# xingyizhou/CenterTrack

Hardware: NVIDIA H100
Metric: frames/sec (device-timed) DLA-34 512x512 (higher is better)
Workload: dtype bf16

## Files before the change

### centertrack_b200/csrc/conv_halo.cu

```cuda
#include "conv_common.cuh"
#include "wgmma.cuh"
#include <cuda.h>
#include <stdlib.h>
#include <string.h>

namespace ctb {

constexpr int HT_W = 8, HT_H = 16;

__device__ unsigned long long* g_halo_trace = nullptr;
__device__ __forceinline__ unsigned long long* h_trace_ptr() {
  unsigned long long* t = g_halo_trace;
  return (t != nullptr && blockIdx.x == 0) ? t : nullptr;
}
__device__ __forceinline__ void h_stamp(unsigned long long* t, int it, int k) {
  if (t != nullptr && it < 256) t[it * 8 + k] = (unsigned long long)clock64();
}
constexpr int H_THREADS = 288;
constexpr int H_MMA_WARPS = 8;
constexpr int H_STAGING_BYTES = 2 * 64 * EPI_PITCH * 4;

struct HaloArgs {
  ConvGeom g;
  const __nv_bfloat16* w;
  const float* shift;
  const __nv_bfloat16* residual;
  void* out;
  int n_tile, n_tiles_n, nblk, planes, pw, ph, plane_bytes, box_bytes, halo_stages;
  int tw, th;
  int tiles_x, tiles_y, tiles_total;
  int pair_taps;
  int swz;
  int merged_xc;
  int out_s2d;
  int sum3;
  uint32_t w_bytes;
  int m_nky, m_nkx, m_nc, m_nq;
  uint32_t m_sky, m_skx, m_sc, m_sq, m_alo, m_ahi;
};

template <int N, bool OVERLAP>
__global__ void __launch_bounds__(H_THREADS, (N <= 128 && !OVERLAP) ? 2 : 1)
conv_halo_kernel(const HaloArgs a, const __grid_constant__ CUtensorMap tmap) {
  extern __shared__ __align__(1024) unsigned char hsm_dyn[];
  unsigned char* sm = hsm_dyn + ((1024u - (smem_u32(hsm_dyn) & 1023u)) & 1023u);
  const ConvGeom& g = a.g;
  const int tid = threadIdx.x, warp = tid >> 5, lane = tid & 31;
  unsigned long long* const trace = h_trace_ptr();
  const int S = a.halo_stages;
  const uint32_t halo_bytes = (uint32_t)a.planes * a.plane_bytes;

  const uint32_t base = smem_u32(sm);
  const uint32_t sW = base;
  const uint32_t sH = base + ((a.w_bytes + 1023u) & ~1023u);
  const uint32_t off_stg = ((a.w_bytes + 1023u) & ~1023u) + S * halo_bytes;
  const uint32_t off_bar = off_stg + H_STAGING_BYTES;
  const uint32_t bars = base + off_bar;
  const uint32_t w_full = bars;
  auto halo_full = [&](int s) { return bars + 8u * (1 + s); };
  auto halo_empty = [&](int s) { return bars + 8u * (1 + S + s); };

  pdl_trigger();
  if (tid == 0) {
    mbar_init(w_full, 1);
    for (int s = 0; s < S; ++s) { mbar_init(halo_full(s), 1); mbar_init(halo_empty(s), H_MMA_WARPS); }
    mbar_init_fence();
  }
  float* s_shift = reinterpret_cast<float*>(sm + off_bar + 256);
  {
    const int n0s = (blockIdx.x % a.n_tiles_n) * N;
    for (int j = tid; j < 256; j += H_THREADS)
      s_shift[j] = (a.shift && j < N && n0s + j < g.C_out) ? __ldg(a.shift + n0s + j) : 0.f;
  }
  __syncthreads();
  if (warp == 8 && lane == 0) {
    mbar_arrive_expect_tx(w_full, a.w_bytes);
    bulk_g2s(sW, reinterpret_cast<const unsigned char*>(a.w) + (size_t)(blockIdx.x % a.n_tiles_n) * a.w_bytes, a.w_bytes, w_full);
  }
  pdl_wait();

  const int nt = blockIdx.x % a.n_tiles_n;
  const int sp0 = blockIdx.x / a.n_tiles_n;
  const int sp_stride = gridDim.x / a.n_tiles_n;
  const int sp_total = a.tiles_total;
  const int n0 = nt * N;
  const int per_img = a.tiles_x * a.tiles_y;

  if (warp == 8) {
    if (lane == 0) {
      int it = 0;
      for (int sp = sp0; sp < sp_total; sp += sp_stride, ++it) {
        const int s = it % S;
        const uint32_t ph = (uint32_t)(it / S) & 1u;
        mbar_wait(halo_empty(s), ph ^ 1u, 1, it);
        h_stamp(trace, it, 0);
        const int b = sp / per_img, r = sp - b * per_img;
        const int ty = r / a.tiles_x, tx = r - ty * a.tiles_x;
        const int x0 = tx * a.tw - g.pad, y0 = ty * a.th - g.pad;
        mbar_arrive_expect_tx(halo_full(s), (uint32_t)(a.planes * a.box_bytes));
        if (a.merged_xc) {
          tma_3d(sH + s * halo_bytes, &tmap, x0 * 8, y0, b, halo_full(s));
        } else {
          const int cstep = a.swz ? (a.swz >> 1) : 8;
          for (int p = 0; p < a.planes; ++p)
            tma_4d(sH + s * halo_bytes + p * a.plane_bytes, &tmap, p * cstep, x0, y0, b, halo_full(s));
        }
        h_stamp(trace, it, 1);
      }
    }
  } else {
    const int wg = warp >> 2, w4 = warp & 3;
    const int lrow = 32 * (w4 & 1) + lane;
    const int chalf = w4 >> 1;
    const int row = 64 * wg + lrow;
    const uint32_t stg = base + off_stg + (uint32_t)wg * (64u * EPI_PITCH * 4u);
    const uint64_t b_desc0 = wg_desc(sW, (uint32_t)N * 16u, 128u, 0u);
    const uint32_t b_step = ((uint32_t)N * 32u) >> 4;
    const uint32_t half16 = (uint32_t)wg * 8u * (a.m_ahi & 0x3FFFu);
    const int gpr = a.tw >> 3;
    const int gy = (row >> 3) / gpr, rx = (((row >> 3) % gpr) << 3) | (row & 7);
    const int HWo = g.OH * g.OW;
    constexpr int PF = 2;
    uint4 rq[PF][2];
    const bool use_res = a.residual != nullptr && g.out_mode == CT_OUT_NHWC && !a.sum3;
    auto prefetch_residual = [&](int sp_n) {
      const int bn = sp_n / per_img, rn = sp_n - bn * per_img;
      const int tyn = rn / a.tiles_x, txn = rn - tyn * a.tiles_x;
      const int oyn = tyn * a.th + gy, oxn = txn * a.tw + rx;
      const bool okn = oyn < g.OH && oxn < g.OW;
      const size_t pn = ((size_t)bn * g.OH + oyn) * g.OW + oxn;
#pragma unroll
      for (int i = 0; i < PF; ++i) {
        const int col = chalf * 16 + 32 * i;
        rq[i][0] = make_uint4(0, 0, 0, 0); rq[i][1] = make_uint4(0, 0, 0, 0);
        if (okn && col < N && n0 + col < g.C_out) {
          const uint4* rp = reinterpret_cast<const uint4*>(a.residual + pn * g.ld_res + n0 + col);
          rq[i][0] = __ldg(rp); rq[i][1] = __ldg(rp + 1);
        }
      }
    };
    if (use_res && sp0 < sp_total) prefetch_residual(sp0);
    mbar_wait(w_full, 0, 2, 0);
    if constexpr (OVERLAP)
      if (wg == 1 && sp0 < sp_total) named_arrive(3, 256);
    float acc[N / 2];
    int it = 0;
    for (int sp = sp0; sp < sp_total; sp += sp_stride, ++it) {
      const int s = it % S;
      const uint32_t ph = (uint32_t)(it / S) & 1u;
      if constexpr (OVERLAP) named_sync(3 + wg, 256);
      mbar_wait(halo_full(s), ph, 3, it);
      if (tid == 0) h_stamp(trace, it, 2);
      const uint32_t a_lo0 = a.m_alo + (sH >> 4) + ((uint32_t)s * halo_bytes >> 4) + half16;
      uint64_t b_desc = b_desc0;
      uint32_t accum = 0;
      wg_fence();
      for (int ky = 0; ky < a.m_nky; ++ky)
        for (int kx = 0; kx < a.m_nkx; ++kx)
          for (int c = 0; c < a.m_nc; ++c)
            for (int qq = 0; qq < a.m_nq; ++qq) {
              const uint32_t a_lo = a_lo0 + (uint32_t)ky * a.m_sky + (uint32_t)kx * a.m_skx + (uint32_t)c * a.m_sc +
                                    (uint32_t)qq * a.m_sq;
              Wgmma<N>::mma(acc, ((uint64_t)a.m_ahi << 32) | (uint64_t)a_lo, b_desc, accum);
              accum = 1;
              b_desc += b_step;
            }
      wg_commit();
      wg_wait<0>();
      wg_fence_operand(acc);
      if constexpr (OVERLAP) named_arrive(3 + (wg ^ 1), 256);
      __syncwarp();
      if (lane == 0) mbar_arrive(halo_empty(s));
      if (tid == 0) h_stamp(trace, it, 4);

      const int b = sp / per_img, r = sp - b * per_img;
      const int ty = r / a.tiles_x, tx = r - ty * a.tiles_x;
      const int oy = ty * a.th + gy, ox = tx * a.tw + rx;
      const bool p_ok = oy < g.OH && ox < g.OW;
      const size_t p = a.out_s2d ? ((((size_t)b * (g.OH >> 1) + (oy >> 1)) * (g.OW >> 1) + (ox >> 1)) << 2) + (((oy & 1) << 1) | (ox & 1))
                                 : ((size_t)b * g.OH + oy) * g.OW + ox;
      if (tid == 0) h_stamp(trace, it, 5);
      float s8[8];
#pragma unroll
      for (int j = 0; j < 8; ++j) s8[j] = 0.f;
#pragma unroll
      for (int c0 = 0; c0 < N; c0 += 32) {
        named_sync(1 + wg, 128);
        stage_acc_chunk(acc, c0, stg, 0);
        named_sync(1 + wg, 128);
        const uint32_t srow = stg + (uint32_t)lrow * EPI_PITCH * 4u;
        if (a.sum3) {
#pragma unroll
          for (int grp = 0; grp < 3; ++grp) {
            if (grp * 16 < c0 || grp * 16 >= c0 + 32 || grp * 16 >= N) continue;
            if (!((a.sum3 >> grp) & 1)) continue;
            float rr[8];
            lds_f(srow + (uint32_t)(grp * 16 - c0 + chalf * 8) * 4u, rr);
            const float4* sh4 = reinterpret_cast<const float4*>(s_shift + grp * 16 + chalf * 8);
            const float4 sa = sh4[0], sb = sh4[1];
            s8[0] += fmaxf(rr[0] + sa.x, 0.f); s8[1] += fmaxf(rr[1] + sa.y, 0.f);
            s8[2] += fmaxf(rr[2] + sa.z, 0.f); s8[3] += fmaxf(rr[3] + sa.w, 0.f);
            s8[4] += fmaxf(rr[4] + sb.x, 0.f); s8[5] += fmaxf(rr[5] + sb.y, 0.f);
            s8[6] += fmaxf(rr[6] + sb.z, 0.f); s8[7] += fmaxf(rr[7] + sb.w, 0.f);
          }
          continue;
        }
        const int col = c0 + chalf * 16;
        const int o0 = n0 + col;
        if (col >= N || !p_ok || o0 >= g.C_out) continue;
        float v[16];
        lds_f(srow + (uint32_t)chalf * 64u, v);
        const float4* sh4 = reinterpret_cast<const float4*>(s_shift + col);
#pragma unroll
        for (int j4 = 0; j4 < 4; ++j4) {
          const float4 sh = sh4[j4];
          v[4 * j4 + 0] += sh.x; v[4 * j4 + 1] += sh.y; v[4 * j4 + 2] += sh.z; v[4 * j4 + 3] += sh.w;
        }
        if (g.out_mode == CT_OUT_NHWC) {
          if (a.residual) {
            uint4 ra, rb;
            const int ci = col >> 5;
            if (ci < PF) {
// ... 56 lines not shown
    if ((g.OH | g.OW) & 1 || d->residual)
      return fail(CT_ERR_INVALID, "conv_halo: CT_OUT_NHWC_S2D needs even OH / OW, no residual%s", "");
    a.out_s2d = 1;
    a.g.out_mode = CT_OUT_NHWC;
  }
  if (a.sum3 && !(g.C_out == 48 && n_tile == 48 && g.out_mode == CT_OUT_NHWC && d->shift))
    return fail(CT_ERR_INVALID, "conv_halo: sum3 epilogue needs C_out == n_tile == 48, NHWC output, shift%s", "");
  if (g.out_mode == CT_OUT_NHWC && !a.sum3 && (g.C_out % 16 != 0 || g.ld_out % 8 != 0))
    return fail(CT_ERR_INVALID, "conv_halo: NHWC bf16 output needs C_out %% 16 == 0, ld_out %% 8 == 0%s", "");
  if (d->residual && (g.out_mode != CT_OUT_NHWC || g.ld_res % 8 != 0))
    return fail(CT_ERR_INVALID, "conv_halo: residual only for NHWC bf16 outputs, ld_res %% 8 == 0%s", "");
  a.n_tile = n_tile;
  a.n_tiles_n = (g.C_out + n_tile - 1) / n_tile;
  a.pair_taps = g.C_in == 8;
  a.nblk = halo_blocks(g.C_in, g.KH, g.KW);
  if (a.nblk > 160) return fail(CT_ERR_UNSUPPORTED, "conv_halo: more than 160 K=16 blocks per tile%s (%ld)", "", (long)a.nblk);
  static const bool force_planes = [] { const char* e = getenv("CTB_HALO_MODE"); return e && strcmp(e, "planes") == 0; }();
  a.swz = (g.C_in > 64) ? 128 : ((!force_planes && (g.C_in == 16 || g.C_in == 32 || g.C_in == 64)) ? g.C_in * 2 : 0);
  a.merged_xc = (g.C_in == 8 && g.ld_in == 8) ? 1 : 0;
  a.planes = a.swz ? (g.C_in * 2 + a.swz - 1) / a.swz : g.C_in / 8;
  a.tw = HT_W; a.th = HT_H;
  static const int wide_env = getenv("CTB_HALO_WIDE") ? atoi(getenv("CTB_HALO_WIDE")) : 1;
  if (wide_env && g.KH == 1 && g.KW == 1 && g.out_mode == CT_OUT_NCHW_F32 && a.swz && g.OW % 32 == 0 && g.OH % 4 == 0) {
    a.tw = 32; a.th = 4;
  }
  a.pw = a.tw + g.KW - 1 + (a.pair_taps ? 1 : 0);
  a.ph = a.th + g.KH - 1;
  a.box_bytes = a.pw * a.ph * (a.swz ? a.swz : 16);
  a.plane_bytes = (a.box_bytes + 1023) / 1024 * 1024;
  a.w_bytes = (uint32_t)a.nblk * n_tile * 32u;
  if (a.pair_taps) {
    a.m_nky = g.KH; a.m_nkx = (g.KW + 1) / 2; a.m_nc = 1; a.m_nq = 1;
    a.m_sky = a.pw; a.m_skx = 2; a.m_sc = 0; a.m_sq = 0;
    a.m_alo = 1u << 16;
    a.m_ahi = (uint32_t)a.pw;
  } else if (a.swz) {
    const uint32_t rb16 = (uint32_t)a.swz >> 4;
    a.m_nky = g.KH; a.m_nkx = g.KW; a.m_nc = a.planes; a.m_nq = (g.C_in < 64 ? g.C_in : 64) / 16;
    a.m_sky = (uint32_t)a.pw * rb16; a.m_skx = rb16; a.m_sc = (uint32_t)a.plane_bytes >> 4; a.m_sq = 2;
    a.m_alo = 1u << 16;
    const uint32_t layout = a.swz == 128 ? 1u : (a.swz == 64 ? 2u : 3u);
    const uint32_t sbo16 = a.tw == HT_W ? (uint32_t)a.pw * rb16 : 8u * rb16;
    a.m_ahi = sbo16 | (layout << 30);
  } else {
    a.m_nky = g.KH; a.m_nkx = g.KW; a.m_nc = 1; a.m_nq = g.C_in / 16;
    a.m_sky = a.pw; a.m_skx = 1; a.m_sc = 0; a.m_sq = 2u * ((uint32_t)a.plane_bytes >> 4);
    a.m_alo = ((uint32_t)a.plane_bytes >> 4) << 16;
    a.m_ahi = (uint32_t)a.pw;
  }
  a.tiles_x = (g.OW + a.tw - 1) / a.tw;
  a.tiles_y = (g.OH + a.th - 1) / a.th;
  a.tiles_total = g.B * a.tiles_x * a.tiles_y;
  const size_t halo_bytes = (size_t)a.planes * a.plane_bytes;
  auto smem_for = [&](int s) { return (size_t)((a.w_bytes + 1023) & ~1023u) + s * halo_bytes + H_STAGING_BYTES + 256 + 1024 + 1024; };
  auto ctas_for = [&](int s) {
    const int n = (int)((227 * 1024) / smem_for(s));
    return n > 2 ? 2 : n;
  };
  int stages = 2;
  for (int sdeep = 4; sdeep >= 3; --sdeep)
    if (smem_for(sdeep) <= 227 * 1024 && ctas_for(sdeep) == ctas_for(2)) { stages = sdeep; break; }
  static const int stages_env = getenv("CTB_HALO_STAGES") ? atoi(getenv("CTB_HALO_STAGES")) : 0;
  if (stages_env >= 2) stages = stages_env;
  if (smem_for(stages) > 227 * 1024)
    return fail(CT_ERR_UNSUPPORTED, "conv_halo: weights + halo do not fit in shared memory%s (%ld bytes)", "",
                (long)smem_for(stages));
  a.halo_stages = stages;
  int per_sm = ctas_for(stages);
  if (n_tile > 128) per_sm = 1;
  static const int overlap_env = getenv("CTB_HALO_OVERLAP") ? atoi(getenv("CTB_HALO_OVERLAP")) : 1;
  c.smem_bytes = (int32_t)smem_for(stages);
  c.stages = stages;
  c.tile_w = a.tw;
  c.tile_h = a.th;
  c.ctas_per_sm = per_sm;
  c.overlap = overlap_env && per_sm == 1 && n_tile >= 64 && n_tile <= 128;
  return CT_OK;
}

int conv_config_halo(const ct_conv_desc* d, ConvConfig* c) {
  HaloArgs a;
  return halo_config(d, a, *c);
}

int conv_forward_halo(const ct_conv_desc* d, cudaStream_t st) {
  HaloArgs a;
  ConvConfig c;
  const int rc = halo_config(d, a, c);
  if (rc != CT_OK) return rc;
  if (((uintptr_t)d->x & 15) || ((uintptr_t)d->w & 15) || ((uintptr_t)d->out & 15) || ((uintptr_t)d->residual & 15))
    return fail(CT_ERR_INVALID, "conv_halo: x/w/out/residual must be 16-byte aligned%s", "");
  a.w = (const __nv_bfloat16*)d->w;
  a.shift = d->shift;
  a.residual = (const __nv_bfloat16*)d->residual;
  a.out = d->out;
  const ConvGeom& g = a.g;

  CUtensorMap tmap;
  int r;
  if (a.merged_xc) {
    const cuuint64_t dims[3] = {(cuuint64_t)g.W * 8, (cuuint64_t)g.H, (cuuint64_t)g.B};
    const cuuint64_t strides[2] = {(cuuint64_t)g.W * 16, (cuuint64_t)g.H * g.W * 16};
    const cuuint32_t box[3] = {(cuuint32_t)a.pw * 8, (cuuint32_t)a.ph, 1};
    r = encode_tmap_bf16(&tmap, d->x, 3, dims, strides, box, CU_TENSOR_MAP_SWIZZLE_NONE);
  } else {
    const cuuint64_t dims[4] = {(cuuint64_t)g.C_in, (cuuint64_t)g.W, (cuuint64_t)g.H, (cuuint64_t)g.B};
    const cuuint64_t strides[3] = {(cuuint64_t)g.ld_in * 2, (cuuint64_t)g.W * g.ld_in * 2,
                                   (cuuint64_t)g.H * g.W * g.ld_in * 2};
    const cuuint32_t box[4] = {(cuuint32_t)(a.swz ? a.swz / 2 : 8), (cuuint32_t)a.pw, (cuuint32_t)a.ph, 1};
    const CUtensorMapSwizzle sw = a.swz == 128 ? CU_TENSOR_MAP_SWIZZLE_128B
                                  : a.swz == 64 ? CU_TENSOR_MAP_SWIZZLE_64B
                                  : a.swz == 32 ? CU_TENSOR_MAP_SWIZZLE_32B : CU_TENSOR_MAP_SWIZZLE_NONE;
    r = encode_tmap_bf16(&tmap, d->x, 4, dims, strides, box, sw);
  }
  if (r != CT_OK) return r;

  const int sms = device_sm_count();
  long want = (long)sms * c.ctas_per_sm;
  long groups = want / a.n_tiles_n;
  if (groups < 1) groups = 1;
  if (groups > a.tiles_total) groups = a.tiles_total;
  const int grid = (int)(groups * a.n_tiles_n);
  return dispatch_n_tile(a.n_tile, [&](auto n) {
    constexpr int NT = decltype(n)::value;
    if constexpr (NT >= 64 && NT <= 128)
      if (c.overlap)
        return launch_big_smem<conv_halo_kernel<NT, true>>(dim3(grid), dim3(H_THREADS), c.smem_bytes, st, a, tmap);
    return launch_big_smem<conv_halo_kernel<NT, false>>(dim3(grid), dim3(H_THREADS), c.smem_bytes, st, a, tmap);
  });
}

}
```

### centertrack_b200/csrc/conv_heads.cu

```cuda
#include "conv_common.cuh"
#include "wgmma.cuh"
#include <cuda.h>

namespace ctb {

constexpr int HD_TW = 8, HD_TH = 16;
constexpr int HD_THREADS = 320;
constexpr int HD_HALO_STAGES = 2;
constexpr int HD_MAX_N2 = 80;
constexpr uint32_t HD_SLOT_BYTES = 16384;
constexpr int HD_STAGING_BYTES = 2 * 64 * EPI_PITCH * 4;

struct HeadArgs {
  ConvGeom g;
  const unsigned char* w1;
  const float* shift;
  int n_heads, halves, w_stages;
  int tiles_x, tiles_y, tiles_total;
  uint32_t halo_bytes, box_bytes;
  uint32_t a_ahi;
  uint32_t a_sky;
  struct Head { const unsigned char* w2; const float* bias; float* out; int c_out, act; } h[CT_MAX_FUSED_HEADS];
};

template <int NH, int N2>
__global__ void __launch_bounds__(HD_THREADS, 1)
conv_heads_kernel(const __grid_constant__ HeadArgs a, const __grid_constant__ CUtensorMap tmap) {
  extern __shared__ __align__(1024) unsigned char hsm_dyn[];
  unsigned char* sm = hsm_dyn + ((1024u - (smem_u32(hsm_dyn) & 1023u)) & 1023u);
  const ConvGeom& g = a.g;
  const int tid = threadIdx.x, warp = tid >> 5, lane = tid & 31;
  const int S = a.w_stages;
  constexpr uint32_t MID_BYTES = 64u * NH * 2u;
  constexpr int KSL = NH / 64;

  const uint32_t base = smem_u32(sm);
  const uint32_t sH = base;
  const uint32_t sW = sH + HD_HALO_STAGES * a.halo_bytes;
  const uint32_t sM = sW + (uint32_t)S * HD_SLOT_BYTES;
  const uint32_t sS = sM + 2u * MID_BYTES;
  const uint32_t bars = sS + HD_STAGING_BYTES;
  auto halo_full = [&](int s) { return bars + 8u * s; };
  auto halo_empty = [&](int s) { return bars + 8u * (HD_HALO_STAGES + s); };
  auto w_full = [&](int s) { return bars + 8u * (2 * HD_HALO_STAGES + s); };
  auto w_empty = [&](int s) { return bars + 8u * (2 * HD_HALO_STAGES + S + s); };

  pdl_trigger();
  if (tid == 0) {
    for (int s = 0; s < HD_HALO_STAGES; ++s) { mbar_init(halo_full(s), 1); mbar_init(halo_empty(s), 8); }
    for (int s = 0; s < S; ++s) { mbar_init(w_full(s), 1); mbar_init(w_empty(s), 8); }
    mbar_init_fence();
  }
  __syncthreads();
  pdl_wait();
  const int per_img = a.tiles_x * a.tiles_y;

  if (warp == 8) {
    if (lane == 0) {
      uint32_t k = 0;
      auto put = [&](const unsigned char* src, uint32_t bytes) {
        const int s = (int)(k % (uint32_t)S);
        mbar_wait(w_empty(s), ((k / (uint32_t)S) & 1u) ^ 1u, 4, (int)k);
        mbar_arrive_expect_tx(w_full(s), bytes);
        bulk_g2s(sW + (uint32_t)s * HD_SLOT_BYTES, src, bytes, w_full(s));
        ++k;
      };
      for (int sp = blockIdx.x; sp < a.tiles_total; sp += gridDim.x)
        for (int h = 0; h < a.n_heads; ++h) {
          for (int j = 0; j < a.halves; ++j) {
            const unsigned char* w1 = a.w1 + (size_t)(h * a.halves + j) * 36 * NH * 32;
            for (int t = 0; t < 9; ++t) put(w1 + t * 4 * NH * 32, 4u * NH * 32u);
            for (int q = 0; q < KSL; ++q) put(a.h[h].w2 + (size_t)(j * KSL + q) * 4 * N2 * 32, 4u * N2 * 32u);
          }
        }
    }
  } else if (warp == 9) {
    if (lane == 0) {
      int it = 0;
      for (int sp = blockIdx.x; sp < a.tiles_total; sp += gridDim.x, ++it) {
        const int s = it % HD_HALO_STAGES;
        mbar_wait(halo_empty(s), ((uint32_t)(it / HD_HALO_STAGES) & 1u) ^ 1u, 5, it);
        const int b = sp / per_img, r = sp - b * per_img;
        const int ty = r / a.tiles_x, tx = r - ty * a.tiles_x;
        mbar_arrive_expect_tx(halo_full(s), a.box_bytes);
        tma_4d(sH + (uint32_t)s * a.halo_bytes, &tmap, 0, tx * HD_TW - 1, ty * HD_TH - 1, b, halo_full(s));
      }
    }
  } else {
    const int wg = warp >> 2, w4 = warp & 3;
    const int lrow = 32 * (w4 & 1) + lane;
    const int chalf = w4 >> 1;
    const int row = 64 * wg + lrow;
    const int gy = row >> 3, rx = row & 7;
    const uint32_t stg = sS + (uint32_t)wg * (64u * EPI_PITCH * 4u);
    const uint32_t mid = sM + (uint32_t)wg * MID_BYTES;
    const int fl = tid & 31, frow = 16 * w4 + (fl >> 2), fcol = 2 * (fl & 3);
    const uint32_t half16 = (uint32_t)wg * 8u * (a.a_ahi & 0x3FFFu);
    const uint64_t a_hi = (uint64_t)a.a_ahi << 32;
    const uint64_t mid_desc = wg_desc(mid, 16u, 1024u, 1u);
    const int HWo = g.OH * g.OW;
    auto release = [&](uint32_t kk, bool pred) {
      __syncwarp();
      mbar_arrive_if(w_empty((int)(kk % (uint32_t)S)), pred && lane == 0);
    };
    float acc[NH / 2];
    float acc2[N2 / 2];
    uint32_t k = 0;
    int it = 0;
    for (int sp = blockIdx.x; sp < a.tiles_total; sp += gridDim.x, ++it) {
      const int hs = it % HD_HALO_STAGES;
      mbar_wait(halo_full(hs), (uint32_t)(it / HD_HALO_STAGES) & 1u, 6, it);
      const uint32_t a_lo0 = (1u << 16) + ((sH + (uint32_t)hs * a.halo_bytes) >> 4) + half16;
      const int b = sp / per_img, r = sp - b * per_img;
      const int ty = r / a.tiles_x, tx = r - ty * a.tiles_x;
      const int oy = ty * HD_TH + gy, ox = tx * HD_TW + rx;
      const bool p_ok = oy < g.OH && ox < g.OW;
      for (int h = 0; h < a.n_heads; ++h) {
        for (int j = 0; j < a.halves; ++j) {
          for (int tap = 0; tap < 9; ++tap, ++k) {
            const int s = (int)(k % (uint32_t)S);
            mbar_wait_inline(w_full(s), (k / (uint32_t)S) & 1u);
            const uint32_t a_lo = a_lo0 + (uint32_t)(tap / 3) * a.a_sky + (uint32_t)(tap % 3) * 8u;
            const uint64_t b_desc = wg_desc(sW + (uint32_t)s * HD_SLOT_BYTES, NH * 16u, 128u, 0u);
            wg_fence();
#pragma unroll
            for (int q = 0; q < 4; ++q)
              Wgmma<NH>::mma(acc, a_hi | (uint64_t)(a_lo + 2u * q), b_desc + (uint64_t)q * ((NH * 32) >> 4),
                             (tap | q) != 0 ? 1u : 0u);
            wg_commit();
            wg_wait<1>();
            release(k - 1, tap > 0);
          }
          wg_wait<0>();
          wg_fence_operand(acc);
          release(k - 1, true);
          mbar_arrive_if(halo_empty(hs), lane == 0 && h == a.n_heads - 1 && j == a.halves - 1);
          const float* sh = a.shift + (size_t)(h * a.halves + j) * NH;
#pragma unroll
          for (int i = 0; i < NH / 8; ++i) {
            const int c = 8 * i + fcol;
            const float s0 = __ldg(sh + c), s1 = __ldg(sh + c + 1);
#pragma unroll
            for (int hh = 0; hh < 2; ++hh) {
              const int rr = frow + 8 * hh;
              const __nv_bfloat162 v = __floats2bfloat162_rn(fmaxf(acc[4 * i + 2 * hh] + s0, 0.f),
                                                            fmaxf(acc[4 * i + 2 * hh + 1] + s1, 0.f));
              const uint32_t addr = mid + (uint32_t)(i >> 3) * 8192u + (uint32_t)rr * 128u +
                                    ((uint32_t)((i & 7) ^ (rr & 7)) << 4) + (uint32_t)fcol * 2u;
              sts32(addr, *reinterpret_cast<const uint32_t*>(&v));
            }
          }
          fence_proxy_async();
          named_sync(1 + wg, 128);
          for (int q = 0; q < KSL; ++q, ++k) {
            const int s = (int)(k % (uint32_t)S);
            mbar_wait_inline(w_full(s), (k / (uint32_t)S) & 1u);
            const uint64_t ad = mid_desc + (uint64_t)(q * (8192 >> 4));
            const uint64_t bd = wg_desc(sW + (uint32_t)s * HD_SLOT_BYTES, N2 * 16u, 128u, 0u);
            wg_fence();
#pragma unroll
            for (int kq = 0; kq < 4; ++kq)
              Wgmma<N2>::mma(acc2, ad + 2u * kq, bd + (uint64_t)kq * ((N2 * 32) >> 4), (j | q | kq) != 0 ? 1u : 0u);
            wg_commit();
          }
          wg_wait<0>();
          wg_fence_operand(acc2);
          for (int q = 0; q < KSL; ++q) release(k - KSL + q, true);
        }
        ConvGeom gh = g;
        gh.C_out = a.h[h].c_out; gh.relu = 0; gh.head_act = a.h[h].act;
        const float* bias = a.h[h].bias;
#pragma unroll
        for (int c0 = 0; c0 < N2; c0 += 32) {
          named_sync(1 + wg, 128);
          stage_acc_chunk(acc2, c0, stg, 0);
          named_sync(1 + wg, 128);
          const int col = c0 + chalf * 16;
          if (col >= N2 || !p_ok || col >= gh.C_out) continue;
          float v[16];
          lds_f(stg + (uint32_t)lrow * EPI_PITCH * 4u + (uint32_t)chalf * 64u, v);
#pragma unroll
          for (int jj = 0; jj < 16; ++jj) v[jj] += col + jj < gh.C_out ? __ldg(bias + col + jj) : 0.f;
          store_head16(a.h[h].out + ((size_t)b * gh.C_out + col) * HWo + (size_t)oy * g.OW + ox, HWo, v, col, gh);
        }
      }
    }
  }
}

static int heads_config(const ct_conv_desc* d, HeadArgs& a, ConvConfig& c) {
  a.g = make_geom(d);
  const ConvGeom& g = a.g;
  if (g.KH != 3 || g.KW != 3 || g.stride != 1 || g.pad != 1 || g.OH != g.H || g.OW != g.W)
    return fail(CT_ERR_INVALID, "fused heads: the shared layer must be a 3x3 stride-1 'same' convolution%s", "");
  if (g.C_in != 64 || g.ld_in % 8 != 0)
    return fail(CT_ERR_INVALID, "fused heads: C_in must be 64 (ld_in %% 8 == 0)%s (%ld)", "", g.C_in);
  if (d->n_heads < 1 || d->n_heads > CT_MAX_FUSED_HEADS || !d->heads)
    return fail(CT_ERR_INVALID, "fused heads: 1 .. 12 heads and a head table%s (%ld)", "", d->n_heads);
  if (g.C_out % d->n_heads != 0 || !(g.C_out / d->n_heads == 64 || g.C_out / d->n_heads == 256))
    return fail(CT_ERR_INVALID, "fused heads: 64 or 256 mid channels per head%s (C_out %ld)", "", g.C_out);
  const int mid_c = g.C_out / d->n_heads;
  if (d->n_tile != (mid_c == 256 ? 128 : 64))
    return fail(CT_ERR_INVALID, "fused heads: n_tile must be 128 (256 mid channels) or 64 (64)%s (%ld)", "", d->n_tile);
  if (g.out_mode != CT_OUT_NCHW_F32 || !g.relu || d->residual || d->epilogue_sum3)
    return fail(CT_ERR_INVALID, "fused heads: fp32 NCHW outputs, ReLU on the 3x3, no residual%s", "");
  a.n_heads = d->n_heads;
  a.halves = mid_c / d->n_tile;
  for (int i = 0; i < d->n_heads; ++i) {
    const ct_head& hd = d->heads[i];
    if (hd.C_out < 1 || hd.n_tile % 16 != 0 || hd.n_tile < hd.C_out || hd.n_tile > HD_MAX_N2 ||
        hd.n_tile != d->heads[0].n_tile)
      return fail(CT_ERR_INVALID, "fused heads: one n_tile for every head, C_out <= n_tile <= 80, n_tile %% 16 == 0%s (head %ld)", "", i);
    a.h[i].c_out = hd.C_out; a.h[i].act = hd.head_act;
    a.h[i].w2 = (const unsigned char*)hd.w; a.h[i].bias = hd.bias; a.h[i].out = hd.out;
  }
  const int pw = HD_TW + 2, ph = HD_TH + 2;
  a.box_bytes = (uint32_t)(pw * ph * 128);
  a.halo_bytes = (a.box_bytes + 1023u) & ~1023u;
  a.a_sky = (uint32_t)pw * 8u;
  a.a_ahi = a.a_sky | (1u << 30);
// ... 60 lines not shown
```

### centertrack_b200/csrc/wgmma.cuh

```cuda
#pragma once
#include "conv_common.cuh"
#include "ptx.cuh"

namespace ctb {

constexpr int EPI_PITCH = 36;

template <int M>
__device__ __forceinline__ void stage_acc_chunk(const float (&d)[M], int c0, uint32_t stg, int row0) {
  const int t = threadIdx.x & 127, w = t >> 5, l = t & 31;
  const uint32_t r = (uint32_t)(row0 + 16 * w + (l >> 2));
#pragma unroll
  for (int i = 0; i < M / 4; ++i) {
    if (i * 8 < c0 || i * 8 >= c0 + 32) continue;
    const uint32_t col = (uint32_t)(i * 8 - c0 + 2 * (l & 3));
    sts_f2(stg + (r * EPI_PITCH + col) * 4u, d[4 * i], d[4 * i + 1]);
    sts_f2(stg + ((r + 8u) * EPI_PITCH + col) * 4u, d[4 * i + 2], d[4 * i + 3]);
  }
}

__device__ __forceinline__ void relu16(float (&v)[16], int relu) {
  if (relu) {
#pragma unroll
    for (int j = 0; j < 16; ++j) v[j] = fmaxf(v[j], 0.f);
// ... 28 lines not shown
      v[4 * j4] += rr.x; v[4 * j4 + 1] += rr.y; v[4 * j4 + 2] += rr.z; v[4 * j4 + 3] += rr.w;
    }
  }
  relu16(v, relu);
  float4* o4 = reinterpret_cast<float4*>(op);
#pragma unroll
  for (int j4 = 0; j4 < 4; ++j4) o4[j4] = make_float4(v[4 * j4], v[4 * j4 + 1], v[4 * j4 + 2], v[4 * j4 + 3]);
}
__device__ __forceinline__ void store_f32_nhwc16(float* op, float (&v)[16], int o0, const ConvGeom& g) {
  relu16(v, g.relu);
#pragma unroll
  for (int j = 0; j < 16; ++j) {
    const float sg = sigmoidf_fast(v[j]);
    v[j] = (o0 + j >= g.sig_from) ? sg : v[j];
  }
  if (o0 + 16 <= g.ld_out && (g.ld_out & 3) == 0) {
#pragma unroll
    for (int j4 = 0; j4 < 4; ++j4)
      reinterpret_cast<float4*>(op)[j4] = make_float4(v[4 * j4], v[4 * j4 + 1], v[4 * j4 + 2], v[4 * j4 + 3]);
  } else {
#pragma unroll
    for (int j = 0; j < 16; ++j) if (o0 + j < g.C_out) op[j] = v[j];
  }
}
__device__ __forceinline__ void store_head16(float* op, size_t plane, float (&v)[16], int o0, const ConvGeom& g) {
  relu16(v, g.relu);
  if (g.head_act == CT_HEAD_SIGMOID) {
#pragma unroll
    for (int j = 0; j < 16; ++j) v[j] = sigmoidf_fast(v[j]);
  } else if (g.head_act == CT_HEAD_DEPTH) {
#pragma unroll
    for (int j = 0; j < 16; ++j) v[j] = (__fdividef(1.f, sigmoidf_fast(v[j]) + 1e-6f) - 1.f) * g.depth_scale;
  }
#pragma unroll
  for (int j = 0; j < 16; ++j)
    if (o0 + j < g.C_out) op[(size_t)j * plane] = v[j];
}

__device__ __forceinline__ void wg_fence() { asm volatile("wgmma.fence.sync.aligned;" ::: "memory"); }
__device__ __forceinline__ void wg_commit() { asm volatile("wgmma.commit_group.sync.aligned;" ::: "memory"); }
template <int PENDING>
__device__ __forceinline__ void wg_wait() { asm volatile("wgmma.wait_group.sync.aligned %0;" ::"n"(PENDING) : "memory"); }
template <int M>
__device__ __forceinline__ void wg_fence_operand(float (&d)[M]) {
#pragma unroll
  for (int i = 0; i < M; ++i) asm volatile("" : "+f"(d[i])::"memory");
}

__device__ __forceinline__ uint64_t wg_desc(uint32_t addr, uint32_t lbo, uint32_t sbo, uint32_t layout) {
  return (uint64_t)((addr & 0x3FFFFu) >> 4) | ((uint64_t)((lbo >> 4) & 0x3FFFu) << 16) |
         ((uint64_t)((sbo >> 4) & 0x3FFFu) << 32) | ((uint64_t)layout << 62);
}

template <int N>
struct Wgmma;

template <>
struct Wgmma<16> {
  static __device__ __forceinline__ void mma(float (&d)[8], uint64_t a, uint64_t b, uint32_t acc) {
    asm volatile(
        "{\n\t.reg .pred p;\n\tsetp.ne.b32 p, %10, 0;\n\t"
        "wgmma.mma_async.sync.aligned.m64n16k16.f32.bf16.bf16 {%0,%1,%2,%3,%4,%5,%6,%7}, %8, %9, p, 1, 1, 0, 0;\n\t}"
        : "+f"(d[0]), "+f"(d[1]), "+f"(d[2]), "+f"(d[3]), "+f"(d[4]), "+f"(d[5]), "+f"(d[6]), "+f"(d[7])
        : "l"(a), "l"(b), "r"(acc));
  }
};

template <>
struct Wgmma<32> {
  static __device__ __forceinline__ void mma(float (&d)[16], uint64_t a, uint64_t b, uint32_t acc) {
    asm volatile(
        "{\n\t.reg .pred p;\n\tsetp.ne.b32 p, %18, 0;\n\t"
        "wgmma.mma_async.sync.aligned.m64n32k16.f32.bf16.bf16 {%0,%1,%2,%3,%4,%5,%6,%7,%8,%9,%10,%11,%12,%13,%14,%15}, %16, %17, p, 1, 1, 0, 0;\n\t}"
        : "+f"(d[0]), "+f"(d[1]), "+f"(d[2]), "+f"(d[3]), "+f"(d[4]), "+f"(d[5]), "+f"(d[6]), "+f"(d[7]), "+f"(d[8]), "+f"(d[9]), "+f"(d[10]), "+f"(d[11]), "+f"(d[12]), "+f"(d[13]), "+f"(d[14]), "+f"(d[15])
        : "l"(a), "l"(b), "r"(acc));
  }
};

template <>
struct Wgmma<48> {
  static __device__ __forceinline__ void mma(float (&d)[24], uint64_t a, uint64_t b, uint32_t acc) {
    asm volatile(
        "{\n\t.reg .pred p;\n\tsetp.ne.b32 p, %26, 0;\n\t"
        "wgmma.mma_async.sync.aligned.m64n48k16.f32.bf16.bf16 {%0,%1,%2,%3,%4,%5,%6,%7,%8,%9,%10,%11,%12,%13,%14,%15,%16,%17,%18,%19,%20,%21,%22,%23}, %24, %25, p, 1, 1, 0, 0;\n\t}"
        : "+f"(d[0]), "+f"(d[1]), "+f"(d[2]), "+f"(d[3]), "+f"(d[4]), "+f"(d[5]), "+f"(d[6]), "+f"(d[7]), "+f"(d[8]), "+f"(d[9]), "+f"(d[10]), "+f"(d[11]), "+f"(d[12]), "+f"(d[13]), "+f"(d[14]), "+f"(d[15]), "+f"(d[16]), "+f"(d[17]), "+f"(d[18]), "+f"(d[19]), "+f"(d[20]), "+f"(d[21]), "+f"(d[22]), "+f"(d[23])
        : "l"(a), "l"(b), "r"(acc));
  }
};

template <>
struct Wgmma<64> {
  static __device__ __forceinline__ void mma(float (&d)[32], uint64_t a, uint64_t b, uint32_t acc) {
    asm volatile(
        "{\n\t.reg .pred p;\n\tsetp.ne.b32 p, %34, 0;\n\t"
        "wgmma.mma_async.sync.aligned.m64n64k16.f32.bf16.bf16 {%0,%1,%2,%3,%4,%5,%6,%7,%8,%9,%10,%11,%12,%13,%14,%15,%16,%17,%18,%19,%20,%21,%22,%23,%24,%25,%26,%27,%28,%29,%30,%31}, %32, %33, p, 1, 1, 0, 0;\n\t}"
        : "+f"(d[0]), "+f"(d[1]), "+f"(d[2]), "+f"(d[3]), "+f"(d[4]), "+f"(d[5]), "+f"(d[6]), "+f"(d[7]), "+f"(d[8]), "+f"(d[9]), "+f"(d[10]), "+f"(d[11]), "+f"(d[12]), "+f"(d[13]), "+f"(d[14]), "+f"(d[15]), "+f"(d[16]), "+f"(d[17]), "+f"(d[18]), "+f"(d[19]), "+f"(d[20]), "+f"(d[21]), "+f"(d[22]), "+f"(d[23]), "+f"(d[24]), "+f"(d[25]), "+f"(d[26]), "+f"(d[27]), "+f"(d[28]), "+f"(d[29]), "+f"(d[30]), "+f"(d[31])
        : "l"(a), "l"(b), "r"(acc));
  }
};

template <>
struct Wgmma<80> {
  static __device__ __forceinline__ void mma(float (&d)[40], uint64_t a, uint64_t b, uint32_t acc) {
    asm volatile(
        "{\n\t.reg .pred p;\n\tsetp.ne.b32 p, %42, 0;\n\t"
        "wgmma.mma_async.sync.aligned.m64n80k16.f32.bf16.bf16 {%0,%1,%2,%3,%4,%5,%6,%7,%8,%9,%10,%11,%12,%13,%14,%15,%16,%17,%18,%19,%20,%21,%22,%23,%24,%25,%26,%27,%28,%29,%30,%31,%32,%33,%34,%35,%36,%37,%38,%39}, %40, %41, p, 1, 1, 0, 0;\n\t}"
// ... 128 lines not shown
```

Baseline: 2419.

## Stream conv_halo weights through a shared-memory ring when full weights don't fit

Adds a RING variant of the halo conv kernel for large-weight layers (128B swizzle, C_in multiple of 64, n_tile 64..128) whose whole weight block plus two halo stages would exceed shared memory. An extra producer warp streams per-tap weight slices into a 4-8 slot mbarrier ring, and the MMA warps consume them slice by slice with wait_group<1> pipelining. This lets such layers run instead of failing or using shallow staging, at the cost of re-fetching weights for every tile, one CTA per SM and no overlap schedule. The heads kernel is refactored to use the shared WeightRing helper.

```diff
diff --git a/centertrack_b200/csrc/conv_halo.cu b/centertrack_b200/csrc/conv_halo.cu
--- a/centertrack_b200/csrc/conv_halo.cu
+++ b/centertrack_b200/csrc/conv_halo.cu
@@ -35,13 +35,17 @@
   int out_s2d;
   int sum3;
   uint32_t w_bytes;
+  int ring, w_stages, w_slices;
+  uint32_t slice_bytes;
   int m_nky, m_nkx, m_nc, m_nq;
   uint32_t m_sky, m_skx, m_sc, m_sq, m_alo, m_ahi;
 };
 
-template <int N, bool OVERLAP>
-__global__ void __launch_bounds__(H_THREADS, (N <= 128 && !OVERLAP) ? 2 : 1)
+template <int N, bool OVERLAP, bool RING>
+__global__ void __launch_bounds__(RING ? H_THREADS + 32 : H_THREADS, (N <= 128 && !OVERLAP && !RING) ? 2 : 1)
 conv_halo_kernel(const HaloArgs a, const __grid_constant__ CUtensorMap tmap) {
+  static_assert(!(OVERLAP && RING), "the streamed-weight flavour runs the serial schedule");
+  constexpr int THREADS = RING ? H_THREADS + 32 : H_THREADS;
   extern __shared__ __align__(1024) unsigned char hsm_dyn[];
   unsigned char* sm = hsm_dyn + ((1024u - (smem_u32(hsm_dyn) & 1023u)) & 1023u);
   const ConvGeom& g = a.g;
@@ -52,32 +56,30 @@
 
   const uint32_t base = smem_u32(sm);
   const uint32_t sW = base;
-  const uint32_t sH = base + ((a.w_bytes + 1023u) & ~1023u);
-  const uint32_t off_stg = ((a.w_bytes + 1023u) & ~1023u) + S * halo_bytes;
+  const uint32_t w_region = ((RING ? (uint32_t)a.w_stages * a.slice_bytes : a.w_bytes) + 1023u) & ~1023u;
+  const uint32_t sH = base + w_region;
+  const uint32_t off_stg = w_region + S * halo_bytes;
   const uint32_t off_bar = off_stg + H_STAGING_BYTES;
   const uint32_t bars = base + off_bar;
   const uint32_t w_full = bars;
   auto halo_full = [&](int s) { return bars + 8u * (1 + s); };
   auto halo_empty = [&](int s) { return bars + 8u * (1 + S + s); };
+  const WeightRing<128u * N> ring{sW, bars + 8u * (1 + 2 * S), (uint32_t)a.w_stages};
 
   pdl_trigger();
   if (tid == 0) {
     mbar_init(w_full, 1);
     for (int s = 0; s < S; ++s) { mbar_init(halo_full(s), 1); mbar_init(halo_empty(s), H_MMA_WARPS); }
+    if constexpr (RING) ring.init();
     mbar_init_fence();
   }
   float* s_shift = reinterpret_cast<float*>(sm + off_bar + 256);
   {
     const int n0s = (blockIdx.x % a.n_tiles_n) * N;
-    for (int j = tid; j < 256; j += H_THREADS)
+    for (int j = tid; j < 256; j += THREADS)
       s_shift[j] = (a.shift && j < N && n0s + j < g.C_out) ? __ldg(a.shift + n0s + j) : 0.f;
   }
   __syncthreads();
-  if (warp == 8 && lane == 0) {
-    mbar_arrive_expect_tx(w_full, a.w_bytes);
-    bulk_g2s(sW, reinterpret_cast<const unsigned char*>(a.w) + (size_t)(blockIdx.x % a.n_tiles_n) * a.w_bytes, a.w_bytes, w_full);
-  }
-  pdl_wait();
 
   const int nt = blockIdx.x % a.n_tiles_n;
   const int sp0 = blockIdx.x / a.n_tiles_n;
@@ -85,6 +87,20 @@
   const int sp_total = a.tiles_total;
   const int n0 = nt * N;
   const int per_img = a.tiles_x * a.tiles_y;
+
+  const unsigned char* const w_nt = reinterpret_cast<const unsigned char*>(a.w) + (size_t)nt * a.w_bytes;
+  if constexpr (RING) {
+    if (warp == 9) {
+      if (lane == 0)
+        for (uint32_t k = 0, sp = sp0; (int)sp < sp_total; sp += sp_stride)
+          for (int j = 0; j < a.w_slices; ++j, ++k) ring.put(k, w_nt + (size_t)j * a.slice_bytes, a.slice_bytes);
+      return;
+    }
+  } else if (warp == 8 && lane == 0) {
+    mbar_arrive_expect_tx(w_full, a.w_bytes);
+    bulk_g2s(sW, w_nt, a.w_bytes, w_full);
+  }
+  pdl_wait();
 
   if (warp == 8) {
     if (lane == 0) {
@@ -140,11 +156,12 @@
       }
     };
     if (use_res && sp0 < sp_total) prefetch_residual(sp0);
-    mbar_wait(w_full, 0, 2, 0);
+    if constexpr (!RING) mbar_wait(w_full, 0, 2, 0);
     if constexpr (OVERLAP)
       if (wg == 1 && sp0 < sp_total) named_arrive(3, 256);
     float acc[N / 2];
     int it = 0;
+    uint32_t k = 0;
     for (int sp = sp0; sp < sp_total; sp += sp_stride, ++it) {
       const int s = it % S;
       const uint32_t ph = (uint32_t)(it / S) & 1u;
@@ -152,22 +169,44 @@
       mbar_wait(halo_full(s), ph, 3, it);
       if (tid == 0) h_stamp(trace, it, 2);
       const uint32_t a_lo0 = a.m_alo + (sH >> 4) + ((uint32_t)s * halo_bytes >> 4) + half16;
-      uint64_t b_desc = b_desc0;
-      uint32_t accum = 0;
-      wg_fence();
-      for (int ky = 0; ky < a.m_nky; ++ky)
-        for (int kx = 0; kx < a.m_nkx; ++kx)
-          for (int c = 0; c < a.m_nc; ++c)
-            for (int qq = 0; qq < a.m_nq; ++qq) {
-              const uint32_t a_lo = a_lo0 + (uint32_t)ky * a.m_sky + (uint32_t)kx * a.m_skx + (uint32_t)c * a.m_sc +
-                                    (uint32_t)qq * a.m_sq;
-              Wgmma<N>::mma(acc, ((uint64_t)a.m_ahi << 32) | (uint64_t)a_lo, b_desc, accum);
-              accum = 1;
-              b_desc += b_step;
+      if constexpr (RING) {
+        int j = 0;
+        for (int ky = 0; ky < a.m_nky; ++ky)
+          for (int kx = 0; kx < a.m_nkx; ++kx)
+            for (int c = 0; c < a.m_nc; ++c, ++j, ++k) {
+              ring.wait(k);
+              const uint32_t a_lo = a_lo0 + (uint32_t)ky * a.m_sky + (uint32_t)kx * a.m_skx + (uint32_t)c * a.m_sc;
+              const uint64_t b_desc = wg_desc(ring.slot(k), (uint32_t)N * 16u, 128u, 0u);
+              wg_fence();
+#pragma unroll
+              for (int qq = 0; qq < 4; ++qq)
+                Wgmma<N>::mma(acc, ((uint64_t)a.m_ahi << 32) | (uint64_t)(a_lo + (uint32_t)qq * a.m_sq),
+                              b_desc + (uint64_t)qq * b_step, (j | qq) != 0 ? 1u : 0u);
+              wg_commit();
+              wg_wait<1>();
+              ring.release(k - 1, j > 0);
             }
-      wg_commit();
-      wg_wait<0>();
-      wg_fence_operand(acc);
+        wg_wait<0>();
+        wg_fence_operand(acc);
+        ring.release(k - 1, true);
+      } else {
+        uint64_t b_desc = b_desc0;
+        uint32_t accum = 0;
+        wg_fence();
+        for (int ky = 0; ky < a.m_nky; ++ky)
+          for (int kx = 0; kx < a.m_nkx; ++kx)
+            for (int c = 0; c < a.m_nc; ++c)
+              for (int qq = 0; qq < a.m_nq; ++qq) {
+                const uint32_t a_lo = a_lo0 + (uint32_t)ky * a.m_sky + (uint32_t)kx * a.m_skx + (uint32_t)c * a.m_sc +
+                                      (uint32_t)qq * a.m_sq;
+                Wgmma<N>::mma(acc, ((uint64_t)a.m_ahi << 32) | (uint64_t)a_lo, b_desc, accum);
+                accum = 1;
+                b_desc += b_step;
+              }
+        wg_commit();
+        wg_wait<0>();
+        wg_fence_operand(acc);
+      }
       if constexpr (OVERLAP) named_arrive(3 + (wg ^ 1), 256);
       __syncwarp();
       if (lane == 0) mbar_arrive(halo_empty(s));
@@ -330,13 +369,30 @@
   a.tiles_y = (g.OH + a.th - 1) / a.th;
   a.tiles_total = g.B * a.tiles_x * a.tiles_y;
   const size_t halo_bytes = (size_t)a.planes * a.plane_bytes;
-  auto smem_for = [&](int s) { return (size_t)((a.w_bytes + 1023) & ~1023u) + s * halo_bytes + H_STAGING_BYTES + 256 + 1024 + 1024; };
+  uint32_t w_region = a.w_bytes;
+  auto smem_for = [&](int s) { return (size_t)((w_region + 1023) & ~1023u) + s * halo_bytes + H_STAGING_BYTES + 256 + 1024 + 1024; };
+  static const int ring_env = getenv("CTB_HALO_RING") ? atoi(getenv("CTB_HALO_RING")) : 1;
+  a.ring = 0;
+  a.w_stages = 0;
+  a.slice_bytes = (uint32_t)a.m_nq * n_tile * 32u;
+  a.w_slices = a.m_nky * a.m_nkx * a.m_nc;
+  if (ring_env && smem_for(2) > 227 * 1024 && a.swz == 128 && g.C_in % 64 == 0 && n_tile >= 64 && n_tile <= 128 &&
+      !a.sum3 && a.tw == HT_W) {
+    for (int ws = 8; ws >= 4 && !a.w_stages; --ws) {
+      w_region = (uint32_t)ws * a.slice_bytes;
+      if (smem_for(2) <= 227 * 1024) a.w_stages = ws;
+    }
+    if (!a.w_stages)
+      return fail(CT_ERR_UNSUPPORTED, "conv_halo: weight ring + halo do not fit in shared memory%s (%ld bytes)", "",
+                  (long)smem_for(2));
+    a.ring = 1;
+  }
   auto ctas_for = [&](int s) {
     const int n = (int)((227 * 1024) / smem_for(s));
     return n > 2 ? 2 : n;
   };
   int stages = 2;
-  for (int sdeep = 4; sdeep >= 3; --sdeep)
+  for (int sdeep = 4; sdeep >= 3 && !a.ring; --sdeep)
     if (smem_for(sdeep) <= 227 * 1024 && ctas_for(sdeep) == ctas_for(2)) { stages = sdeep; break; }
   static const int stages_env = getenv("CTB_HALO_STAGES") ? atoi(getenv("CTB_HALO_STAGES")) : 0;
   if (stages_env >= 2) stages = stages_env;
@@ -345,14 +401,14 @@
                 (long)smem_for(stages));
   a.halo_stages = stages;
   int per_sm = ctas_for(stages);
-  if (n_tile > 128) per_sm = 1;
+  if (n_tile > 128 || a.ring) per_sm = 1;
   static const int overlap_env = getenv("CTB_HALO_OVERLAP") ? atoi(getenv("CTB_HALO_OVERLAP")) : 1;
   c.smem_bytes = (int32_t)smem_for(stages);
   c.stages = stages;
   c.tile_w = a.tw;
   c.tile_h = a.th;
   c.ctas_per_sm = per_sm;
-  c.overlap = overlap_env && per_sm == 1 && n_tile >= 64 && n_tile <= 128;
+  c.overlap = overlap_env && per_sm == 1 && n_tile >= 64 && n_tile <= 128 && !a.ring;
   return CT_OK;
 }
 
@@ -401,10 +457,13 @@
   const int grid = (int)(groups * a.n_tiles_n);
   return dispatch_n_tile(a.n_tile, [&](auto n) {
     constexpr int NT = decltype(n)::value;
-    if constexpr (NT >= 64 && NT <= 128)
+    if constexpr (NT >= 64 && NT <= 128) {
+      if (a.ring)
+        return launch_big_smem<conv_halo_kernel<NT, false, true>>(dim3(grid), dim3(H_THREADS + 32), c.smem_bytes, st, a, tmap);
       if (c.overlap)
-        return launch_big_smem<conv_halo_kernel<NT, true>>(dim3(grid), dim3(H_THREADS), c.smem_bytes, st, a, tmap);
-    return launch_big_smem<conv_halo_kernel<NT, false>>(dim3(grid), dim3(H_THREADS), c.smem_bytes, st, a, tmap);
+        return launch_big_smem<conv_halo_kernel<NT, true, false>>(dim3(grid), dim3(H_THREADS), c.smem_bytes, st, a, tmap);
+    }
+    return launch_big_smem<conv_halo_kernel<NT, false, false>>(dim3(grid), dim3(H_THREADS), c.smem_bytes, st, a, tmap);
   });
 }
 
diff --git a/centertrack_b200/csrc/conv_heads.cu b/centertrack_b200/csrc/conv_heads.cu
--- a/centertrack_b200/csrc/conv_heads.cu
+++ b/centertrack_b200/csrc/conv_heads.cu
@@ -40,15 +40,14 @@
   const uint32_t sM = sW + (uint32_t)S * HD_SLOT_BYTES;
   const uint32_t sS = sM + 2u * MID_BYTES;
   const uint32_t bars = sS + HD_STAGING_BYTES;
-  auto halo_full = [&](int s) { return bars + 8u * s; };
-  auto halo_empty = [&](int s) { return bars + 8u * (HD_HALO_STAGES + s); };
-  auto w_full = [&](int s) { return bars + 8u * (2 * HD_HALO_STAGES + s); };
-  auto w_empty = [&](int s) { return bars + 8u * (2 * HD_HALO_STAGES + S + s); };
+  const WeightRing<HD_SLOT_BYTES> ring{sW, bars, (uint32_t)S};
+  auto halo_full = [&](int s) { return bars + 8u * (2 * S + s); };
+  auto halo_empty = [&](int s) { return bars + 8u * (2 * S + HD_HALO_STAGES + s); };
 
   pdl_trigger();
   if (tid == 0) {
     for (int s = 0; s < HD_HALO_STAGES; ++s) { mbar_init(halo_full(s), 1); mbar_init(halo_empty(s), 8); }
-    for (int s = 0; s < S; ++s) { mbar_init(w_full(s), 1); mbar_init(w_empty(s), 8); }
+    ring.init();
     mbar_init_fence();
   }
   __syncthreads();
@@ -58,13 +57,7 @@
   if (warp == 8) {
     if (lane == 0) {
       uint32_t k = 0;
-      auto put = [&](const unsigned char* src, uint32_t bytes) {
-        const int s = (int)(k % (uint32_t)S);
-        mbar_wait(w_empty(s), ((k / (uint32_t)S) & 1u) ^ 1u, 4, (int)k);
-        mbar_arrive_expect_tx(w_full(s), bytes);
-        bulk_g2s(sW + (uint32_t)s * HD_SLOT_BYTES, src, bytes, w_full(s));
-        ++k;
-      };
+      auto put = [&](const unsigned char* src, uint32_t bytes) { ring.put(k++, src, bytes); };
       for (int sp = blockIdx.x; sp < a.tiles_total; sp += gridDim.x)
         for (int h = 0; h < a.n_heads; ++h) {
           for (int j = 0; j < a.halves; ++j) {
@@ -99,10 +92,6 @@
     const uint64_t a_hi = (uint64_t)a.a_ahi << 32;
     const uint64_t mid_desc = wg_desc(mid, 16u, 1024u, 1u);
     const int HWo = g.OH * g.OW;
-    auto release = [&](uint32_t kk, bool pred) {
-      __syncwarp();
-      mbar_arrive_if(w_empty((int)(kk % (uint32_t)S)), pred && lane == 0);
-    };
     float acc[NH / 2];
     float acc2[N2 / 2];
     uint32_t k = 0;
@@ -118,10 +107,9 @@
       for (int h = 0; h < a.n_heads; ++h) {
         for (int j = 0; j < a.halves; ++j) {
           for (int tap = 0; tap < 9; ++tap, ++k) {
-            const int s = (int)(k % (uint32_t)S);
-            mbar_wait_inline(w_full(s), (k / (uint32_t)S) & 1u);
+            ring.wait(k);
             const uint32_t a_lo = a_lo0 + (uint32_t)(tap / 3) * a.a_sky + (uint32_t)(tap % 3) * 8u;
-            const uint64_t b_desc = wg_desc(sW + (uint32_t)s * HD_SLOT_BYTES, NH * 16u, 128u, 0u);
+            const uint64_t b_desc = wg_desc(ring.slot(k), NH * 16u, 128u, 0u);
             wg_fence();
 #pragma unroll
             for (int q = 0; q < 4; ++q)
@@ -129,11 +117,11 @@
                              (tap | q) != 0 ? 1u : 0u);
             wg_commit();
             wg_wait<1>();
-            release(k - 1, tap > 0);
+            ring.release(k - 1, tap > 0);
           }
           wg_wait<0>();
           wg_fence_operand(acc);
-          release(k - 1, true);
+          ring.release(k - 1, true);
           mbar_arrive_if(halo_empty(hs), lane == 0 && h == a.n_heads - 1 && j == a.halves - 1);
           const float* sh = a.shift + (size_t)(h * a.halves + j) * NH;
 #pragma unroll
@@ -153,10 +141,9 @@
           fence_proxy_async();
           named_sync(1 + wg, 128);
           for (int q = 0; q < KSL; ++q, ++k) {
-            const int s = (int)(k % (uint32_t)S);
-            mbar_wait_inline(w_full(s), (k / (uint32_t)S) & 1u);
+            ring.wait(k);
             const uint64_t ad = mid_desc + (uint64_t)(q * (8192 >> 4));
-            const uint64_t bd = wg_desc(sW + (uint32_t)s * HD_SLOT_BYTES, N2 * 16u, 128u, 0u);
+            const uint64_t bd = wg_desc(ring.slot(k), N2 * 16u, 128u, 0u);
             wg_fence();
 #pragma unroll
             for (int kq = 0; kq < 4; ++kq)
@@ -165,7 +152,7 @@
           }
           wg_wait<0>();
           wg_fence_operand(acc2);
-          for (int q = 0; q < KSL; ++q) release(k - KSL + q, true);
+          for (int q = 0; q < KSL; ++q) ring.release(k - KSL + q, true);
         }
         ConvGeom gh = g;
         gh.C_out = a.h[h].c_out; gh.relu = 0; gh.head_act = a.h[h].act;
diff --git a/centertrack_b200/csrc/wgmma.cuh b/centertrack_b200/csrc/wgmma.cuh
--- a/centertrack_b200/csrc/wgmma.cuh
+++ b/centertrack_b200/csrc/wgmma.cuh
@@ -104,6 +104,29 @@
          ((uint64_t)((sbo >> 4) & 0x3FFFu) << 32) | ((uint64_t)layout << 62);
 }
 
+template <uint32_t SLOT_BYTES>
+struct WeightRing {
+  uint32_t slots;
+  uint32_t bars;
+  uint32_t S;
+  __device__ __forceinline__ uint32_t full(uint32_t k) const { return bars + 8u * (k % S); }
+  __device__ __forceinline__ uint32_t empty(uint32_t k) const { return bars + 8u * (S + k % S); }
+  __device__ __forceinline__ uint32_t slot(uint32_t k) const { return slots + (k % S) * SLOT_BYTES; }
+  __device__ __forceinline__ void init() const {
+    for (uint32_t s = 0; s < S; ++s) { mbar_init(full(s), 1); mbar_init(empty(s), 8); }
+  }
+  __device__ __forceinline__ void put(uint32_t k, const void* src, uint32_t bytes) const {
+    mbar_wait(empty(k), ((k / S) & 1u) ^ 1u, 4, (int)k);
+    mbar_arrive_expect_tx(full(k), bytes);
+    bulk_g2s(slot(k), src, bytes, full(k));
+  }
+  __device__ __forceinline__ void wait(uint32_t k) const { mbar_wait_inline(full(k), (k / S) & 1u); }
+  __device__ __forceinline__ void release(uint32_t k, bool pred) const {
+    __syncwarp();
+    mbar_arrive_if(empty(k), pred && (threadIdx.x & 31) == 0);
+  }
+};
+
 template <int N>
 struct Wgmma;
 
```

After: 2505 (median of 6 runs). +3.5%, better.
